# tmathis720/kryst

Hardware: AMD Instinct MI355X
Metric: cg_iterations_per_sec (higher is better)
Workload: dtype f64; 1 GPU; cg_poisson7_512^3; grid=512, rows=134217728, nnz=937951232, partition=1 k-slab(s), rhs=A*1, x0=0, spmv_encoding=csr-p16, launcher=SoloGroup

## Files before the change

### bindings/rust/src/ffi.rs

```rust
#![allow(non_camel_case_types, dead_code)]
use std::os::raw::{c_char, c_void};

pub type Ctx = *mut c_void;
pub type Csr = *mut c_void;
pub type Vecd = *mut c_void;
pub type Pc = *mut c_void;
pub type Session = *mut c_void;
pub type HostFactors = *mut c_void;
pub type HostAmg = *mut c_void;

pub const KRYST_OK: i32 = 0;
pub const KRYST_FACTOR_ERROR: i32 = 1;
pub const KRYST_SOLVE_ERROR: i32 = 2;
pub const KRYST_INDEFINITE_MATRIX: i32 = 3;
pub const KRYST_INDEFINITE_PRECONDITIONER: i32 = 4;
pub const KRYST_ZERO_PIVOT: i32 = 5;
pub const KRYST_UNSUPPORTED: i32 = 6;
pub const KRYST_ERR_HIP: i32 = 100;
pub const KRYST_ERR_RCCL: i32 = 101;
pub const KRYST_ERR_ARG: i32 = 102;
pub const KRYST_ERR_CSR: i32 = 103;
pub const KRYST_ERR_BUSY: i32 = 104;

pub const KRYST_ILU_KRYST_COMPAT: i32 = 0;
// ... 47 lines not shown
    pub fn kryst_ctx_synchronize(ctx: Ctx) -> i32;
    pub fn kryst_ctx_rank(ctx: Ctx, rank: *mut i32, nranks: *mut i32) -> i32;
    pub fn kryst_comm_barrier(ctx: Ctx) -> i32;
    pub fn kryst_comm_all_reduce(ctx: Ctx, x: f64, out: *mut f64) -> i32;
    pub fn kryst_ctx_scalar_reduce(ctx: Ctx, mode: i32, active: *mut i32) -> i32;
    pub fn kryst_csr_halo_mode(a: Csr, mode: i32, active: *mut i32) -> i32;
    pub fn kryst_ctx_trim(ctx: Ctx, bytes_released: *mut i64) -> i32;
    pub fn kryst_phase_timing_begin(ctx: Ctx) -> i32;
    pub fn kryst_phase_timing_end(ctx: Ctx, ms: *mut f64, count: i32) -> i32;
    pub fn kryst_phase_count() -> i32;
    pub fn kryst_phase_name(phase: i32) -> *const c_char;
    pub fn kryst_ctx_timer_start(ctx: Ctx) -> i32;
    pub fn kryst_ctx_timer_stop(ctx: Ctx, ms: *mut f64) -> i32;

    pub fn kryst_vec_create(ctx: Ctx, n: i64, out: *mut Vecd) -> i32;
    pub fn kryst_vec_destroy(v: Vecd) -> i32;
    pub fn kryst_vec_len(v: Vecd, n: *mut i64) -> i32;
    pub fn kryst_vec_upload(v: Vecd, host: *const f64, n: i64) -> i32;
    pub fn kryst_vec_download(v: Vecd, host: *mut f64, n: i64) -> i32;
    pub fn kryst_vec_fill(v: Vecd, value: f64) -> i32;
    pub fn kryst_vec_copy(dst: Vecd, src: Vecd) -> i32;
    pub fn kryst_vec_fill_splitmix(v: Vecd, seed: u64, global_offset: i64) -> i32;

    pub fn kryst_csr_create(ctx: Ctx, nrows: i64, ncols: i64, row_ptr: *const u64, col_idx: *const u64, vals: *const f64, out: *mut Csr) -> i32;
    pub fn kryst_csr_create_i32(ctx: Ctx, nrows: i64, ncols: i64, row_ptr: *const i64, col_idx: *const i32, vals: *const f64, out: *mut Csr) -> i32;
    pub fn kryst_csr_create_dist(ctx: Ctx, n_global: i64, row_offsets: *const i64, row_ptr: *const i64, col_idx_global: *const i64,
                                 vals: *const f64, out: *mut Csr) -> i32;
    pub fn kryst_csr_create_stencil7(ctx: Ctx, n: i32, kind: i32, out: *mut Csr) -> i32;
    pub fn kryst_csr_destroy(a: Csr) -> i32;
    pub fn kryst_csr_shape(a: Csr, nrows_local: *mut i64, ncols_global: *mut i64, nnz_local: *mut i64) -> i32;
    pub fn kryst_csr_encoding(a: Csr, encoding: *mut i32, patterns: *mut i32, table_entries: *mut i32) -> i32;
    pub fn kryst_csr_tile_order(a: Csr, info: *mut i64) -> i32;
    pub fn kryst_csr_pattern_info(a: Csr, info: *mut i64) -> i32;
    pub fn kryst_csr_download(a: Csr, row_ptr: *mut i64, col_idx_local: *mut i32, vals: *mut f64) -> i32;
    pub fn kryst_csr_placement_info(a: Csr, tries: *mut i32, chosen: *mut i32, skeleton_ms8: *mut f64) -> i32;

    pub fn kryst_spmv(a: Csr, x: Vecd, y: Vecd) -> i32;
    pub fn kryst_spmv_transpose(a: Csr, x: Vecd, y: Vecd) -> i32;
    pub fn kryst_spmv_host(a: Csr, x: *const f64, nx: i64, y: *mut f64, ny: i64) -> i32;
    pub fn kryst_bench_spmv(a: Csr, x: Vecd, y: Vecd, fused_dots: i32, reps: i32, avg_ms: *mut f64) -> i32;
    pub fn kryst_bench_streams(ctx: Ctx, n: i64, stride_bytes: i64, kind: i32, reps: i32, avg_ms: *mut f64) -> i32;
    pub fn kryst_bench_csr_skeleton(a: Csr, x: Vecd, y: Vecd, reps: i32, avg_ms: *mut f64) -> i32;
    pub fn kryst_bench_spmv_fused(a: Csr, x: Vecd, y: Vecd, reps: i32, avg_ms: *mut f64) -> i32;
    pub fn kryst_bench_poison_lds(ctx: Ctx) -> i32;
    pub fn kryst_bench_vec_padding(v: Vecd, fill: *const f64, dirty: *mut i64) -> i32;

    pub fn kryst_dot(x: Vecd, y: Vecd, out: *mut f64) -> i32;
    pub fn kryst_norm(x: Vecd, out: *mut f64) -> i32;
    pub fn kryst_axpy(alpha: f64, x: Vecd, y: Vecd) -> i32;
    pub fn kryst_aypx(beta: f64, x: Vecd, y: Vecd) -> i32;
    pub fn kryst_sub(a: Vecd, b: Vecd, out: Vecd) -> i32;

    pub fn kryst_pc_identity(ctx: Ctx, out: *mut Pc) -> i32;
    pub fn kryst_pc_jacobi(a: Csr, out: *mut Pc) -> i32;
    pub fn kryst_pc_ilu0(a: Csr, mode: i32, out: *mut Pc) -> i32;
    pub fn kryst_pc_ilup(a: Csr, fill: i32, out: *mut Pc) -> i32;
    pub fn kryst_pc_ilut(a: Csr, fill: i32, droptol: f64, out: *mut Pc) -> i32;
    pub fn kryst_pc_chebyshev_stub(ctx: Ctx, degree: i32, out: *mut Pc) -> i32;
    pub fn kryst_pc_chebyshev(a: Csr, alpha: f64, beta: f64, degree: i32, out: *mut Pc) -> i32;
    pub fn kryst_pc_approx_inverse(m: Csr, out: *mut Pc) -> i32;
    pub fn kryst_pc_block_jacobi(a: Csr, blk_ptr: *const i64, blk_idx: *const i64, nblocks: i64, out: *mut Pc) -> i32;
    pub fn kryst_pc_block_jacobi_uniform(a: Csr, bsize: i32, out: *mut Pc) -> i32;
    pub fn kryst_pc_block_jacobi_export(pc: Pc, nnz: *mut i64, row_ptr: *mut i64, col: *mut i32, val: *mut f64) -> i32;
    pub fn kryst_pc_asm(a: Csr, sub_ptr: *const i64, sub_idx: *const i64, nsub: i64, overlap: i32, variant: i32, out: *mut Pc) -> i32;
    pub fn kryst_pc_asm_uniform(a: Csr, nparts: i64, overlap: i32, variant: i32, out: *mut Pc) -> i32;
    pub fn kryst_pc_asm_info(pc: Pc, nsub: *mut i64, ext_rows: *mut i64, max_rows: *mut i32) -> i32;
// ... 73 lines not shown
```

### include/kryst_hip.h

```cpp
#ifndef KRYST_HIP_H
#define KRYST_HIP_H
#include <stdint.h>

#ifdef __cplusplus
extern "C" {
#endif

enum {
    KRYST_OK = 0,
    KRYST_FACTOR_ERROR = 1,
    KRYST_SOLVE_ERROR = 2,
    KRYST_INDEFINITE_MATRIX = 3,
    KRYST_INDEFINITE_PRECONDITIONER = 4,
    KRYST_ZERO_PIVOT = 5,
    KRYST_UNSUPPORTED = 6,
    KRYST_ERR_HIP = 100,
    KRYST_ERR_RCCL = 101,
    KRYST_ERR_ARG = 102,
    KRYST_ERR_CSR = 103,
    KRYST_ERR_BUSY = 104
};

typedef struct kryst_ctx_s* kryst_ctx_t;
typedef struct kryst_csr_s* kryst_csr_t;
// ... 17 lines not shown
int32_t kryst_comm_all_reduce(kryst_ctx_t ctx, double x, double* out);
int32_t kryst_ctx_scalar_reduce(kryst_ctx_t ctx, int32_t mode, int32_t* active);
int32_t kryst_csr_halo_mode(kryst_csr_t a, int32_t mode, int32_t* active);
int32_t kryst_ctx_trim(kryst_ctx_t ctx, int64_t* bytes_released);
int32_t kryst_phase_timing_begin(kryst_ctx_t ctx);
int32_t kryst_phase_timing_end(kryst_ctx_t ctx, double* ms, int32_t count);
int32_t kryst_phase_count(void);
const char* kryst_phase_name(int32_t phase);
int32_t kryst_ctx_timer_start(kryst_ctx_t ctx);
int32_t kryst_ctx_timer_stop(kryst_ctx_t ctx, double* ms);

int32_t kryst_vec_create(kryst_ctx_t ctx, int64_t n, kryst_vec_t* out);
int32_t kryst_vec_destroy(kryst_vec_t v);
int32_t kryst_vec_len(kryst_vec_t v, int64_t* n);
int32_t kryst_vec_upload(kryst_vec_t v, const double* host, int64_t n);
int32_t kryst_vec_download(kryst_vec_t v, double* host, int64_t n);
int32_t kryst_vec_fill(kryst_vec_t v, double value);
int32_t kryst_vec_copy(kryst_vec_t dst, kryst_vec_t src);
int32_t kryst_vec_fill_splitmix(kryst_vec_t v, uint64_t seed, int64_t global_offset);

int32_t kryst_csr_create(kryst_ctx_t ctx, int64_t nrows, int64_t ncols, const uint64_t* row_ptr,
                         const uint64_t* col_idx, const double* vals, kryst_csr_t* out);
int32_t kryst_csr_create_i32(kryst_ctx_t ctx, int64_t nrows, int64_t ncols, const int64_t* row_ptr,
                             const int32_t* col_idx, const double* vals, kryst_csr_t* out);
int32_t kryst_csr_create_dist(kryst_ctx_t ctx, int64_t n_global, const int64_t* row_offsets ,
                              const int64_t* row_ptr, const int64_t* col_idx_global, const double* vals,
                              kryst_csr_t* out);
int32_t kryst_csr_create_stencil7(kryst_ctx_t ctx, int32_t N, int32_t kind, kryst_csr_t* out);
int32_t kryst_csr_destroy(kryst_csr_t a);
int32_t kryst_csr_shape(kryst_csr_t a, int64_t* nrows_local, int64_t* ncols_global, int64_t* nnz_local);
int32_t kryst_csr_encoding(kryst_csr_t a, int32_t* encoding, int32_t* patterns, int32_t* table_entries);
int32_t kryst_csr_tile_order(kryst_csr_t a, int64_t* info);
int32_t kryst_csr_pattern_info(kryst_csr_t a, int64_t* info);
int32_t kryst_csr_download(kryst_csr_t a, int64_t* row_ptr, int32_t* col_idx_local, double* vals);
int32_t kryst_csr_placement_info(kryst_csr_t a, int32_t* tries, int32_t* chosen, double* skeleton_ms8);

int32_t kryst_spmv(kryst_csr_t a, kryst_vec_t x, kryst_vec_t y);
int32_t kryst_spmv_transpose(kryst_csr_t a, kryst_vec_t x, kryst_vec_t y);
int32_t kryst_spmv_host(kryst_csr_t a, const double* x, int64_t nx, double* y, int64_t ny);

int32_t kryst_bench_spmv(kryst_csr_t a, kryst_vec_t x, kryst_vec_t y, int32_t fused_dots, int32_t reps, double* avg_ms);
int32_t kryst_bench_streams(kryst_ctx_t ctx, int64_t n, int64_t stride_bytes, int32_t kind, int32_t reps, double* avg_ms);
int32_t kryst_bench_csr_skeleton(kryst_csr_t a, kryst_vec_t x, kryst_vec_t y, int32_t reps, double* avg_ms);
int32_t kryst_bench_spmv_fused(kryst_csr_t a, kryst_vec_t x, kryst_vec_t y, int32_t reps, double* avg_ms);
int32_t kryst_bench_poison_lds(kryst_ctx_t ctx);
int32_t kryst_bench_vec_padding(kryst_vec_t v, const double* fill, int64_t* dirty);

int32_t kryst_dot(kryst_vec_t x, kryst_vec_t y, double* out);
int32_t kryst_norm(kryst_vec_t x, double* out);
int32_t kryst_axpy(double alpha, kryst_vec_t x, kryst_vec_t y);
int32_t kryst_aypx(double beta, kryst_vec_t x, kryst_vec_t y);
int32_t kryst_sub(kryst_vec_t a, kryst_vec_t b, kryst_vec_t out);

enum { KRYST_ILU_KRYST_COMPAT = 0,
       KRYST_ILU_ILUP0 = 1,
       KRYST_ILU_TRUE_ILU0 = 2 };
int32_t kryst_pc_identity(kryst_ctx_t ctx, kryst_pc_t* out);
int32_t kryst_pc_jacobi(kryst_csr_t a, kryst_pc_t* out);
int32_t kryst_pc_ilu0(kryst_csr_t a, int32_t mode, kryst_pc_t* out);
int32_t kryst_pc_ilup(kryst_csr_t a, int32_t fill, kryst_pc_t* out);
int32_t kryst_pc_ilut(kryst_csr_t a, int32_t fill, double droptol, kryst_pc_t* out);
int32_t kryst_pc_chebyshev_stub(kryst_ctx_t ctx, int32_t degree, kryst_pc_t* out);
int32_t kryst_pc_chebyshev(kryst_csr_t a, double alpha, double beta, int32_t degree, kryst_pc_t* out);
int32_t kryst_pc_approx_inverse(kryst_csr_t m, kryst_pc_t* out);
int32_t kryst_pc_block_jacobi(kryst_csr_t a, const int64_t* blk_ptr, const int64_t* blk_idx, int64_t nblocks, kryst_pc_t* out);
int32_t kryst_pc_block_jacobi_uniform(kryst_csr_t a, int32_t bsize, kryst_pc_t* out);
// ... 123 lines not shown
```

### kryst_amd/__init__.py

```python
import ctypes as C
import enum
import numpy as np

from . import _ffi
from ._ffi import KError, lib, check

__all__ = ["Context", "DeviceVec", "CsrMatrix", "dot", "norm", "Jacobi", "Ilu0", "Ilup", "Ilut", "TrueIlu0", "Chebyshev",
           "ChebyshevPc", "IdentityPc", "ApproxInv", "BlockJacobi", "AdditiveSchwarz", "Sor", "MatSorType", "SparsityPattern", "Spai", "Amg", "apply_chebyshev", "Convergence", "SolveStats", "CgNormType",
           "Preconditioning", "CgSolver", "PcgSolver", "GmresSolver", "FgmresSolver", "PcaGmresSolver", "Orthog", "CgsSolver", "TfqmrSolver", "MinresSolver", "QmrSolver", "CgnrSolver", "CgneSolver", "BiCgStabSolver", "BiCgStabRightPcSolver", "Session", "KspContext", "SolverKind", "PC", "KError", "reduce_spec",
           "host_stencil7", "partition_rows", "halo_recv_plan", "read_matrix_market", "read_petsc_binary", "host_ilup", "host_ilut", "host_amg", "host_levels", "color_graph", "build_blocks_from_colors"]


def _dp(a):
    return a.ctypes.data_as(_ffi.c_dp)


def _f64(a):
    return np.ascontiguousarray(a, dtype=np.float64)


def reduce_spec():
    t, v, f = C.c_int32(), C.c_int32(), C.c_int32()
    lib().kryst_reduce_spec(C.byref(t), C.byref(v), C.byref(f))
    return t.value, v.value, f.value
# ... 250 lines not shown

    def spmv_transpose(self, x, y=None):
        if isinstance(x, DeviceVec):
            if y is None:
                y = DeviceVec(self.ctx, self._ncols)
            check(lib().kryst_spmv_transpose(self.h, x.h, y.h))
            return y
        xv = DeviceVec(self.ctx, _f64(x))
        yv = DeviceVec(self.ctx, self._ncols)
        check(lib().kryst_spmv_transpose(self.h, xv.h, yv.h))
        if y is None:
            return yv.to_host()
        if len(y) != self._ncols:
            raise KError(102, "spmv_transpose: y.len() != ncols")
        y[:] = yv.to_host()
        return y

    ENCODINGS = ("csr", "csr-d8", "csr-d16", "csr-p16", "csr-dia")

    def encoding(self):
        e, p, t = C.c_int32(0), C.c_int32(0), C.c_int32(0)
        check(lib().kryst_csr_encoding(self.h, C.byref(e), C.byref(p), C.byref(t)))
        return self.ENCODINGS[e.value], p.value, t.value

    def tile_order(self):
        info = (C.c_int64 * 4)()
        check(lib().kryst_csr_tile_order(self.h, info))
        return {"plane_rows": info[0], "slots": info[1], "slots8": info[2], "in_use": bool(info[3])}

    def pattern_info(self):
        info = (C.c_int64 * 4)()
        check(lib().kryst_csr_pattern_info(self.h, info))
        return {"line": info[0], "uniform_far": bool(info[1]), "interior_first": info[2], "staged": bool(info[3])}

    def placement_info(self):
        t, c = C.c_int32(0), C.c_int32(0)
        ms = (C.c_double * 8)()
        check(lib().kryst_csr_placement_info(self.h, C.byref(t), C.byref(c), ms))
        return {"tries": t.value, "chosen": c.value, "skeleton_ms": [ms[k] for k in range(t.value)]}

    def bench_spmv(self, x, y, fused_dots=1, reps=50):
        ms = C.c_double()
        check(lib().kryst_bench_spmv(self.h, x.h, y.h, fused_dots, reps, C.byref(ms)))
        return ms.value

    def bench_spmv_fused(self, x, y, reps=20):
        ms = C.c_double()
        rc = lib().kryst_bench_spmv_fused(self.h, x.h, y.h, reps, C.byref(ms))
        if rc == 6:
            return None
        check(rc)
        return ms.value

    def halo_mode(self, mode):
        active = C.c_int32(0)
        rc = lib().kryst_csr_halo_mode(self.h, {"rccl": 0, "peer": 1, "query": -1}[mode], C.byref(active))
        if rc not in (0, 6):
            check(rc)
        return "peer" if active.value == 1 else "rccl"

    def bench_csr_skeleton(self, x, y, reps=10):
        ms = C.c_double()
        check(lib().kryst_bench_csr_skeleton(self.h, x.h, y.h, reps, C.byref(ms)))
        return ms.value

    matvec = spmv
# ... 1075 lines not shown
```

### kryst_amd/_ffi.py

```python
import ctypes as C
import os

_HERE = os.path.dirname(os.path.abspath(__file__))
LIB_PATH = os.environ.get("KRYST_HIP_LIB") or os.path.join(_HERE, "lib", "libkryst_hip.so")

OK = 0
ERR_NAMES = {1: "FactorError", 2: "SolveError", 3: "IndefiniteMatrix", 4: "IndefinitePreconditioner",
             5: "ZeroPivot", 6: "Unsupported", 100: "HipError", 101: "RcclError", 102: "ArgumentError",
             103: "CsrError", 104: "ContextBusy"}

c_dp = C.POINTER(C.c_double)
c_i64p = C.POINTER(C.c_int64)
c_u64p = C.POINTER(C.c_uint64)
c_i32p = C.POINTER(C.c_int32)
Handle = C.c_void_p
MONITOR = C.CFUNCTYPE(None, C.c_int64, C.c_double, C.c_void_p)


class Params(C.Structure):
    _fields_ = [("tol", C.c_double), ("max_iters", C.c_int64), ("restart", C.c_int32),
                ("precond_side", C.c_int32), ("norm_type", C.c_int32), ("single_reduction", C.c_int32),
                ("has_radius", C.c_int32), ("radius", C.c_double),
                ("has_obj_target", C.c_int32), ("obj_target", C.c_double), ("check_every", C.c_int32)]

# ... 19 lines not shown
    "kryst_comm_barrier": (C.c_int32, [Handle]),
    "kryst_comm_all_reduce": (C.c_int32, [Handle, C.c_double, c_dp]),
    "kryst_ctx_scalar_reduce": (C.c_int32, [Handle, C.c_int32, c_i32p]),
    "kryst_csr_halo_mode": (C.c_int32, [Handle, C.c_int32, c_i32p]),
    "kryst_ctx_trim": (C.c_int32, [Handle, c_i64p]),
    "kryst_phase_timing_begin": (C.c_int32, [Handle]),
    "kryst_phase_timing_end": (C.c_int32, [Handle, c_dp, C.c_int32]),
    "kryst_phase_count": (C.c_int32, []),
    "kryst_phase_name": (C.c_char_p, [C.c_int32]),
    "kryst_ctx_timer_start": (C.c_int32, [Handle]),
    "kryst_ctx_timer_stop": (C.c_int32, [Handle, c_dp]),
    "kryst_vec_create": (C.c_int32, [Handle, C.c_int64, C.POINTER(Handle)]),
    "kryst_vec_destroy": (C.c_int32, [Handle]),
    "kryst_vec_len": (C.c_int32, [Handle, c_i64p]),
    "kryst_vec_upload": (C.c_int32, [Handle, c_dp, C.c_int64]),
    "kryst_vec_download": (C.c_int32, [Handle, c_dp, C.c_int64]),
    "kryst_vec_fill": (C.c_int32, [Handle, C.c_double]),
    "kryst_vec_copy": (C.c_int32, [Handle, Handle]),
    "kryst_vec_fill_splitmix": (C.c_int32, [Handle, C.c_uint64, C.c_int64]),
    "kryst_csr_create": (C.c_int32, [Handle, C.c_int64, C.c_int64, c_u64p, c_u64p, c_dp, C.POINTER(Handle)]),
    "kryst_csr_create_i32": (C.c_int32, [Handle, C.c_int64, C.c_int64, c_i64p, c_i32p, c_dp, C.POINTER(Handle)]),
    "kryst_csr_create_dist": (C.c_int32, [Handle, C.c_int64, c_i64p, c_i64p, c_i64p, c_dp, C.POINTER(Handle)]),
    "kryst_csr_create_stencil7": (C.c_int32, [Handle, C.c_int32, C.c_int32, C.POINTER(Handle)]),
    "kryst_csr_destroy": (C.c_int32, [Handle]),
    "kryst_csr_shape": (C.c_int32, [Handle, c_i64p, c_i64p, c_i64p]),
    "kryst_csr_download": (C.c_int32, [Handle, c_i64p, c_i32p, c_dp]),
    "kryst_csr_placement_info": (C.c_int32, [Handle, c_i32p, c_i32p, c_dp]),
    "kryst_spmv": (C.c_int32, [Handle, Handle, Handle]),
    "kryst_spmv_host": (C.c_int32, [Handle, c_dp, C.c_int64, c_dp, C.c_int64]),
    "kryst_spmv_transpose": (C.c_int32, [Handle, Handle, Handle]),
    "kryst_csr_encoding": (C.c_int32, [Handle, C.POINTER(C.c_int32), C.POINTER(C.c_int32), C.POINTER(C.c_int32)]),
    "kryst_csr_tile_order": (C.c_int32, [Handle, C.POINTER(C.c_int64)]),
    "kryst_csr_pattern_info": (C.c_int32, [Handle, C.POINTER(C.c_int64)]),
    "kryst_bench_spmv": (C.c_int32, [Handle, Handle, Handle, C.c_int32, C.c_int32, c_dp]),
    "kryst_bench_streams": (C.c_int32, [Handle, C.c_int64, C.c_int64, C.c_int32, C.c_int32, c_dp]),
    "kryst_bench_csr_skeleton": (C.c_int32, [Handle, Handle, Handle, C.c_int32, c_dp]),
    "kryst_bench_spmv_fused": (C.c_int32, [Handle, Handle, Handle, C.c_int32, c_dp]),
    "kryst_bench_poison_lds": (C.c_int32, [Handle]),
    "kryst_bench_vec_padding": (C.c_int32, [Handle, c_dp, c_i64p]),
    "kryst_dot": (C.c_int32, [Handle, Handle, c_dp]),
    "kryst_norm": (C.c_int32, [Handle, c_dp]),
    "kryst_axpy": (C.c_int32, [C.c_double, Handle, Handle]),
    "kryst_aypx": (C.c_int32, [C.c_double, Handle, Handle]),
    "kryst_sub": (C.c_int32, [Handle, Handle, Handle]),
    "kryst_pc_identity": (C.c_int32, [Handle, C.POINTER(Handle)]),
    "kryst_pc_jacobi": (C.c_int32, [Handle, C.POINTER(Handle)]),
    "kryst_pc_ilu0": (C.c_int32, [Handle, C.c_int32, C.POINTER(Handle)]),
    "kryst_pc_ilup": (C.c_int32, [Handle, C.c_int32, C.POINTER(Handle)]),
    "kryst_pc_ilut": (C.c_int32, [Handle, C.c_int32, C.c_double, C.POINTER(Handle)]),
    "kryst_pc_chebyshev_stub": (C.c_int32, [Handle, C.c_int32, C.POINTER(Handle)]),
    "kryst_pc_chebyshev": (C.c_int32, [Handle, C.c_double, C.c_double, C.c_int32, C.POINTER(Handle)]),
    "kryst_pc_approx_inverse": (C.c_int32, [Handle, C.POINTER(Handle)]),
    "kryst_pc_block_jacobi": (C.c_int32, [Handle, c_i64p, c_i64p, C.c_int64, C.POINTER(Handle)]),
    "kryst_pc_block_jacobi_uniform": (C.c_int32, [Handle, C.c_int32, C.POINTER(Handle)]),
    "kryst_pc_block_jacobi_export": (C.c_int32, [Handle, c_i64p, c_i64p, c_i32p, c_dp]),
    "kryst_pc_asm": (C.c_int32, [Handle, c_i64p, c_i64p, C.c_int64, C.c_int32, C.c_int32, C.POINTER(Handle)]),
    "kryst_pc_asm_uniform": (C.c_int32, [Handle, C.c_int64, C.c_int32, C.c_int32, C.POINTER(Handle)]),
    "kryst_pc_asm_info": (C.c_int32, [Handle, c_i64p, c_i64p, c_i32p]),
    "kryst_pc_asm_export": (C.c_int32, [Handle, c_i64p, c_i32p, c_i32p, c_dp]),
    "kryst_pc_sor": (C.c_int32, [Handle, C.c_double, C.c_int64, C.c_int64, C.c_uint32, C.c_double, c_i32p, C.POINTER(Handle)]),
    "kryst_pc_sor_info": (C.c_int32, [Handle, c_i32p, c_i32p, c_i64p, c_i32p, c_i32p]),
    "kryst_pc_spai": (C.c_int32, [Handle, C.c_int32, c_i64p, c_i64p, C.c_int64, C.c_double, C.POINTER(Handle)]),
    "kryst_pc_spai_export": (C.c_int32, [Handle, c_i64p, c_i64p, c_i32p, c_dp]),
    "kryst_pc_amg": (C.c_int32, [Handle, C.c_int32, C.c_double, C.c_int32, C.c_int32, C.c_int32, C.POINTER(Handle)]),
    "kryst_pc_amg_info": (C.c_int32, [Handle, c_i32p, c_i64p, c_i64p, C.c_int32]),
    "kryst_pc_amg_export": (C.c_int32, [Handle, C.c_int32, C.c_int32, c_i64p, c_i64p, c_i64p, c_i64p, c_i32p, c_dp]),
# ... 111 lines not shown
```

### kryst_amd/csrc/spmv.hip

```cpp
#include "csr.h"
#include "ew.h"
#include <algorithm>


namespace kr {

typedef int    v2i __attribute__((ext_vector_type(2)));
typedef double v2d __attribute__((ext_vector_type(2)));

struct SpmvArgs {
    const int32_t* row_ptr; const int32_t* col; const double* val;
    const double* x; const double* halo; int32_t nloc;
    double* y; const int32_t* tiles; int32_t ntiles; int32_t nrows;
    const double* dvec; double* partials; int64_t pstride;
    const int* done; int32_t xcd_chunk; int32_t swizzle; int32_t group;
    const uint8_t* code; const int32_t* dict;
    const uint16_t* code16; const double* vdict;
    const uint16_t* pid; const uint32_t* pmeta; const int32_t* poff; const double* pval; int32_t npat, ntab;
    int32_t pat_red_off;
    int32_t nloc8;
    int32_t tpw;
    int32_t amask;
    const double* dia; int64_t dia_stride; int32_t dia_nd; int32_t dia_min;
    int64_t xsafe; int32_t cmax;
// ... 595 lines not shown
        if constexpr (NQ > 0) {
            double acc[NQ];
            d2 d;
            if constexpr (CENTER) { d.a = B.x; d.b = B.y; } else d = dv[k];
            acc[0] = 0.0;
            if (va) acc[0] = acc[0] + d.a * s0;
            if (vb) acc[0] = acc[0] + d.b * s1;
            if constexpr (NQ > 1) {
                acc[1] = 0.0;
                if (va) acc[1] = acc[1] + s0 * s0;
                if (vb) acc[1] = acc[1] + s1 * s1;
            }
#pragma unroll
            for (int kk = 0; kk < NQ; ++kk) {
                const double wsum = wave_butterfly(acc[kk]);
                if ((t & 63) == 0) red[(k * NQ + kk) * (KR_T / 64) + (t >> 6)] = wsum;
            }
        }
    }
    if constexpr (NQ > 0) {
        __syncthreads();
        if (t < nt * NQ) {
            const int k = t / NQ, kk = t % NQ;
            double sum = red[t * (KR_T / 64)];
#pragma unroll
            for (int w2 = 1; w2 < KR_T / 64; ++w2) sum = sum + red[t * (KR_T / 64) + w2];
            a.partials[kk * a.pstride + q0 + k] = sum;
        }
    }
}

struct FuseArgs { const double* z; const double* p_old; double* p_new; double* xvec; const double* alpha; const double* beta; const long long* xpend; long long it; };
template <int NQ, int T, int NMAX, bool XU>
__global__ __launch_bounds__(KR_T) void spmv_pattern_fuse_kernel(const SpmvArgs a, const FuseArgs f, const int32_t n, const int32_t far_lo, const int32_t far_hi) {
    const bool ended = a.done && *a.done;
    const bool owed = XU && *f.xpend == f.it - 1;
    if (ended && !owed) return;
    extern __shared__ __attribute__((aligned(16))) unsigned char smem[];
    const int XS = T * KR_TILE + 2 * n + 4;
    double* xs = reinterpret_cast<double*>(smem);
    uint2* meta = reinterpret_cast<uint2*>(xs + XS);
    double* pval = reinterpret_cast<double*>(meta + a.npat);
    double* red = reinterpret_cast<double*>(smem + a.pat_red_off);
    const int t = threadIdx.x;
    const int xcd = blockIdx.x & 7, slot = blockIdx.x >> 3;
    const int G = a.group;
    const int qr = (((slot / G) * 8 + xcd) * G + slot % G) * T;
    if (qr >= a.ntiles) return;
    const int nt = min(T, a.ntiles - qr);
    const int q0 = qr;
    const int32_t r0 = q0 * KR_TILE;
    const double al = *f.alpha, be = *f.beta;
    if (ended) {
#pragma unroll
        for (int k = 0; k < T; ++k) {
            if (k >= nt) break;
            const int32_t row = r0 + k * KR_TILE + 2 * t;
            const d2 pp = ld2(f.p_old, row), xx = ld2(f.xvec, row);
            st2(f.xvec, row, xx.a + al * pp.a, xx.b + al * pp.b);
        }
        return;
    }
    unsigned ids[T];
#pragma unroll
    for (int k = 0; k < T; ++k) ids[k] = k < nt ? __builtin_nontemporal_load(reinterpret_cast<const unsigned*>(a.pid + (size_t)(q0 + k) * KR_TILE + 2 * t)) : 0u;
    constexpr int NP = (T * KR_TILE + 2 * NMAX + 4 + 2 * KR_T - 1) / (2 * KR_T);
    const int npairs = XS / 2;
    const int32_t e0 = r0 - n - 2;
    const int32_t xsafe = (int32_t)a.xsafe;
    const bool inside = e0 >= 0 && e0 + XS <= xsafe && (int64_t)r0 + far_lo >= 0 && (int64_t)r0 + T * KR_TILE + far_hi <= (int64_t)xsafe;
    const int own_lo = (n + 2) / 2, own_hi = own_lo + nt * (KR_TILE / 2);
// ... 610 lines not shown
        a->halo_pushed_inline = inl;
        a->halo_started_for = x;
        return KRYST_OK;
    }
    KR_HIP(hipEventRecord(ctx->ev_x_ready, ctx->s_main));
    KR_HIP(hipStreamWaitEvent(ctx->s_comm, ctx->ev_x_ready, 0));
    const void* sendbase = pl.d_sendbuf;
    if (a->send_contiguous) {
        sendbase = x;
    } else if (pl.total_send > 0) {
        hipLaunchKernelGGL(pack_kernel, dim3((unsigned)((pl.total_send + 255) / 256)), dim3(256), 0, ctx->s_comm,
                           x, pl.d_send_idx, pl.d_sendbuf, pl.total_send);
        KR_HIP(hipGetLastError());
    }
    KR_TRY(comm_exchange(ctx, sendbase, pl.send_counts.data(), pl.send_off.data(), pl.d_halo, pl.recv_counts.data(),
                         pl.recv_off.data(), true, ctx->s_comm));
    KR_HIP(hipEventRecord(ctx->ev_halo_done, ctx->s_comm));
    a->halo_started_for = x;
    return KRYST_OK;
}

bool spmv_can_fuse_direction(kryst_csr_t a) {
    return !a->dist && a->d_pid && a->pat_stage_n > 0 && a->pat_far_uniform && a->npat <= 512 && a->ntab <= 512 && a->nrows == a->xlen &&
           takes_pattern_path(a, false) && env_int("KRYST_SPMV_STAGE", 1) != 0 && env_int("KRYST_SPMV_STAGE_UFAR", 1) != 0 &&
           a->xlen + 2 * KR_TILE < (1ll << 31) &&
           env_int("KRYST_CG_FUSE_P", a->nrows * 8 > env_ll("KRYST_CG_FUSE_MIN_BYTES", 768ll << 20) ? 1 : 0) != 0;
}
static int32_t launch_spmv_fused_impl(kryst_csr_t a, const double* z, const double* p_old, double* p_new, double* xvec, double* y, int nq,
                                      const double* alpha, const double* beta, const long long* xpend, long long it, const int* done, bool force);
int32_t launch_spmv_fused(kryst_csr_t a, const double* z, const double* p_old, double* p_new, double* xvec, double* y, int nq,
                          const double* alpha, const double* beta, const long long* xpend, long long it, const int* done) {
    return launch_spmv_fused_impl(a, z, p_old, p_new, xvec, y, nq, alpha, beta, xpend, it, done, false);
}
static int32_t launch_spmv_fused_impl(kryst_csr_t a, const double* z, const double* p_old, double* p_new, double* xvec, double* y, int nq,
                                      const double* alpha, const double* beta, const long long* xpend, long long it, const int* done, bool force) {
    kryst_ctx_t ctx = a->ctx;
    KR_ARG((force || spmv_can_fuse_direction(a)) && nq >= 1 && nq <= 2, "launch_spmv_fused: operator cannot take the fused form");
    KR_TRY(ensure_partials(ctx, a->ntiles));
    SpmvArgs args;
    memset(&args, 0, sizeof args);
    args.x = p_new; args.y = y; args.ntiles = (int32_t)a->ntiles; args.nrows = (int32_t)a->nrows; args.nloc = (int32_t)a->nrows;
    args.dvec = p_new; args.partials = ctx->d_partials; args.pstride = ctx->partials_cap; args.done = done;
    args.pid = a->d_pid; args.pmeta = a->d_pmeta; args.poff = a->d_poff; args.pval = a->d_pval; args.npat = a->npat; args.ntab = a->ntab;
    const int T = env_int("KRYST_SPMV_FUSE_T", 4) <= 2 ? 2 : 4;
    const int32_t n_ = a->pat_stage_n;
    const size_t xs_bytes = sizeof(double) * (size_t)(T * KR_TILE + 2 * n_ + 4);
    const size_t tab = xs_bytes + (size_t)a->npat * 8 + (size_t)a->ntab * 8;
    args.pat_red_off = (int32_t)((tab + 15) & ~(size_t)15);
    size_t lds_s = (size_t)args.pat_red_off + sizeof(double) * (size_t)T * (size_t)nq * (KR_T / 64);
    const int wgcu = env_int("KRYST_SPMV_FUSE_WG_PER_CU", 0);
    if (wgcu > 0) lds_s = std::max(lds_s, std::min<size_t>((size_t)(160 << 10) / (size_t)wgcu - 512, (size_t)64 << 10));
    args.xsafe = (a->xlen + KR_TILE - 1) / KR_TILE * KR_TILE + KR_TILE - 2;
    const int64_t nruns = (a->ntiles + T - 1) / T;
    args.group = std::max(1, env_int("KRYST_SPMV_STAGE_GROUP", stage_group_default(a, nruns, T, true)));
    const int64_t per_xcd = ((nruns + 7) / 8 + args.group - 1) / args.group * args.group;
    const dim3 sgrid((unsigned)(per_xcd * 8)), block(KR_T);
    const FuseArgs f{z, p_old, p_new, xvec, alpha, beta, xpend, it};
#ifdef KR_TUNING
    args.abl = env_int("KRYST_FUSE_ABL", 0);
#endif
    if (lds_s > ((size_t)48 << 10)) {
        static bool raised = false;
        if (!raised) {
#define KR_FUSE_FNS(NQ_, T_, X_) (const void*)spmv_pattern_fuse_kernel<NQ_, T_, 512, X_>, (const void*)spmv_pattern_fuse_kernel<NQ_, T_, 1024, X_>
            for (const void* fn : {KR_FUSE_FNS(1, 2, true), KR_FUSE_FNS(1, 4, true), KR_FUSE_FNS(2, 2, true), KR_FUSE_FNS(2, 4, true),
                                   KR_FUSE_FNS(1, 2, false), KR_FUSE_FNS(1, 4, false), KR_FUSE_FNS(2, 2, false), KR_FUSE_FNS(2, 4, false)})
                (void)hipFuncSetAttribute(fn, hipFuncAttributeMaxDynamicSharedMemorySize, 64 << 10);
#undef KR_FUSE_FNS
            raised = true;
        }
    }
#define KR_FUSE_N(NQ_, T_, X_) do { if (n_ <= 512) hipLaunchKernelGGL((spmv_pattern_fuse_kernel<NQ_, T_, 512, X_>), sgrid, block, lds_s, ctx->s_main, args, f, n_, a->pat_far_lo, a->pat_far_hi); \
                                    else hipLaunchKernelGGL((spmv_pattern_fuse_kernel<NQ_, T_, 1024, X_>), sgrid, block, lds_s, ctx->s_main, args, f, n_, a->pat_far_lo, a->pat_far_hi); } while (0)
#define KR_FUSE(NQ_) do { if (xvec) { if (T == 2) KR_FUSE_N(NQ_, 2, true); else KR_FUSE_N(NQ_, 4, true); } \
                          else { if (T == 2) KR_FUSE_N(NQ_, 2, false); else KR_FUSE_N(NQ_, 4, false); } } while (0)
    if (nq == 1) KR_FUSE(1); else KR_FUSE(2);
#undef KR_FUSE
#undef KR_FUSE_N
    KR_HIP(hipGetLastError());
    phase_mark(ctx, KR_PH_SPMV);
    return KRYST_OK;
}

static int32_t halo_finish(kryst_csr_t a, int budget) {
    kryst_ctx_t ctx = a->ctx;
    if (a->plan.peer.on) {
        HaloPeer& hp = a->plan.peer;
        if (!a->halo_pushed_inline) KR_HIP(hipStreamWaitEvent(ctx->s_main, ctx->ev_halo_done, 0));
        if (hp.npull > 0) {
            static const int dflt = [] { const char* e = getenv("KRYST_IPC_POLL_BUDGET"); return e ? std::max(1, atoi(e)) : (1 << 26); }();
            const unsigned gx = (unsigned)std::min<int64_t>(std::max<int64_t>(1, (hp.pull_max + 1023) / 1024), 256);
            hipLaunchKernelGGL(halo_pull_kernel, dim3(gx, (unsigned)hp.npull), dim3(256), 0, ctx->s_main, hp.landing + (size_t)(hp.epoch & 1ull) * hp.stride,
                               a->plan.d_halo, hp.d_pull, hp.epoch, budget > 0 ? std::min(budget, dflt) : dflt, fold_err(ctx) + 1);
// ... 62 lines not shown
}

int32_t kryst_spmv(kryst_csr_t a, kryst_vec_t x, kryst_vec_t y) {
    KR_ARG(a && x && y, "spmv");
    KR_ARG(x->ctx == a->ctx && y->ctx == a->ctx, "spmv: context mismatch");
    KR_ARG(x->n == a->xlen, "spmv: x.len() != ncols");
    KR_ARG(y->n == a->nrows, "spmv: y.len() != nrows");
    KR_ARG(x->d != y->d, "spmv: x and y alias");
    KR_HIP(hipSetDevice(a->ctx->device));
    KR_TRY(launch_spmv(a, x->d, y->d, 0, nullptr, nullptr));
    if (a->dist && a->plan.peer.on && use_collectives(a->ctx) && fold_gave_up(a->ctx)) return KRYST_ERR_RCCL;
    return KRYST_OK;
}

int32_t kryst_csr_encoding(kryst_csr_t a, int32_t* encoding, int32_t* patterns, int32_t* table_entries) {
    KR_ARG(a && encoding, "csr_encoding");
    const int lvl = env_int("KRYST_SPMV_COMPRESS", 3);
    int e = 0;
    const bool p16_fits = a->xlen + a->plan.total_recv < (1ll << 28) && a->nrows < (1ll << 28);
    if (a->d_pid && lvl >= 3 && p16_fits) e = 3;
    else if (a->d_code16 && lvl >= 2) e = 2;
    else if (a->d_dia && lvl >= 1 && env_int("KRYST_SPMV_DIA", 1) != 0) e = 4;
    else if (a->d_code && lvl >= 1) e = 1;
    *encoding = e;
    if (patterns) *patterns = e == 4 ? a->dia_nd : (a->d_pid ? a->npat : 0);
    if (table_entries) *table_entries = a->d_pid ? a->ntab : 0;
    return KRYST_OK;
}

int32_t kryst_csr_tile_order(kryst_csr_t a, int64_t* info) {
    KR_ARG(a && info, "csr_tile_order");
    info[0] = a->d_tile_order ? a->order_plane : 0; info[1] = a->order_slots1; info[2] = a->order_slots8;
    info[3] = uses_tile_order(a) ? 1 : 0;
    return KRYST_OK;
}

int32_t kryst_csr_pattern_info(kryst_csr_t a, int64_t* info) {
    KR_ARG(a && info, "csr_pattern_info");
    info[0] = a->d_pid ? a->pat_stage_n : 0; info[1] = a->pat_far_uniform ? 1 : 0; info[2] = a->interior_first;
    info[3] = (a->d_pid && a->pat_stage_n > 0 && takes_pattern_path(a, false) && a->npat <= 512 && a->ntab <= 512 && env_int("KRYST_SPMV_STAGE", 1) != 0 &&
               a->xlen + 2 * KR_TILE < (1ll << 31) && (!a->dist || !use_collectives(a->ctx) || a->interior_first >= 0)) ? 1 : 0;
    return KRYST_OK;
}

int32_t kryst_bench_spmv(kryst_csr_t a, kryst_vec_t x, kryst_vec_t y, int32_t fused_dots, int32_t reps, double* avg_ms) {
    KR_ARG(a && x && y && avg_ms && reps >= 1 && fused_dots >= 0 && fused_dots <= 2, "bench_spmv");
    KR_ARG(x->n == a->xlen && y->n == a->nrows, "bench_spmv: size mismatch");
    KR_ARG(fused_dots == 0 || a->nrows == a->xlen, "bench_spmv: fused dots need a square operator");
    kryst_ctx_t ctx = a->ctx;
    KR_HIP(hipSetDevice(ctx->device));
    const size_t bytes = sizeof(double) * (size_t)((x->n + KR_TILE - 1) / KR_TILE * KR_TILE + KR_TILE);
    double* xs[3] = {x->d, nullptr, nullptr};
    for (int k = 1; k < 3; ++k) {
        if (hipMalloc(&xs[k], bytes) != hipSuccess) { (void)hipGetLastError(); xs[k] = x->d; continue; }
        KR_HIP(hipMemcpyAsync(xs[k], x->d, bytes, hipMemcpyDeviceToDevice, ctx->s_main));
    }
    int32_t rc = launch_spmv(a, xs[0], y->d, fused_dots, xs[0], nullptr);
    (void)hipEventRecord(ctx->tm0, ctx->s_main);
    for (int r = 0; r < reps && rc == KRYST_OK; ++r) rc = launch_spmv(a, xs[(r + 1) % 3], y->d, fused_dots, xs[(r + 1) % 3], nullptr);
    (void)hipEventRecord(ctx->tm1, ctx->s_main);
    (void)hipEventSynchronize(ctx->tm1);
    float ms = 0.f;
    (void)hipEventElapsedTime(&ms, ctx->tm0, ctx->tm1);
    *avg_ms = (double)ms / reps;
    (void)hipStreamSynchronize(ctx->s_main);
    if (use_collectives(ctx)) (void)hipStreamSynchronize(ctx->s_comm);
// ... 53 lines not shown
```

Before: 609.5 iterations/s.

## Add plane-marching fused SpMV kernel reusing z-plane windows in LDS

Adds a marching variant of the fused CG SpMV kernel. Each workgroup owns a strip of a k-plane and walks S consecutive planes, keeping a double-buffered LDS window of the recomputed p vector. The k-1 and k+1 neighbours come from registers and the next plane's window, so the p/z halo for the z-direction is not reloaded. It is enabled by default for large uniform-stencil operators, at the cost of more LDS, fewer workgroups and an extra barrier per plane.

```diff
diff --git a/bindings/rust/src/ffi.rs b/bindings/rust/src/ffi.rs
--- a/bindings/rust/src/ffi.rs
+++ b/bindings/rust/src/ffi.rs
@@ -103,6 +103,7 @@
     pub fn kryst_csr_encoding(a: Csr, encoding: *mut i32, patterns: *mut i32, table_entries: *mut i32) -> i32;
     pub fn kryst_csr_tile_order(a: Csr, info: *mut i64) -> i32;
     pub fn kryst_csr_pattern_info(a: Csr, info: *mut i64) -> i32;
+    pub fn kryst_csr_fuse_march_info(a: Csr, info: *mut i64) -> i32;
     pub fn kryst_csr_download(a: Csr, row_ptr: *mut i64, col_idx_local: *mut i32, vals: *mut f64) -> i32;
     pub fn kryst_csr_placement_info(a: Csr, tries: *mut i32, chosen: *mut i32, skeleton_ms8: *mut f64) -> i32;
 
diff --git a/include/kryst_hip.h b/include/kryst_hip.h
--- a/include/kryst_hip.h
+++ b/include/kryst_hip.h
@@ -73,6 +73,7 @@
 int32_t kryst_csr_encoding(kryst_csr_t a, int32_t* encoding, int32_t* patterns, int32_t* table_entries);
 int32_t kryst_csr_tile_order(kryst_csr_t a, int64_t* info);
 int32_t kryst_csr_pattern_info(kryst_csr_t a, int64_t* info);
+int32_t kryst_csr_fuse_march_info(kryst_csr_t a, int64_t* info);
 int32_t kryst_csr_download(kryst_csr_t a, int64_t* row_ptr, int32_t* col_idx_local, double* vals);
 int32_t kryst_csr_placement_info(kryst_csr_t a, int32_t* tries, int32_t* chosen, double* skeleton_ms8);
 
diff --git a/kryst_amd/__init__.py b/kryst_amd/__init__.py
--- a/kryst_amd/__init__.py
+++ b/kryst_amd/__init__.py
@@ -306,6 +306,11 @@
         info = (C.c_int64 * 4)()
         check(lib().kryst_csr_pattern_info(self.h, info))
         return {"line": info[0], "uniform_far": bool(info[1]), "interior_first": info[2], "staged": bool(info[3])}
+
+    def fuse_march_info(self):
+        info = (C.c_int64 * 6)()
+        check(lib().kryst_csr_fuse_march_info(self.h, info))
+        return {"eligible": bool(info[0]), "on": bool(info[1]), "T": info[2], "strips": info[3], "S": info[4], "segments": info[5]}
 
     def placement_info(self):
         t, c = C.c_int32(0), C.c_int32(0)
diff --git a/kryst_amd/_ffi.py b/kryst_amd/_ffi.py
--- a/kryst_amd/_ffi.py
+++ b/kryst_amd/_ffi.py
@@ -75,6 +75,7 @@
     "kryst_csr_encoding": (C.c_int32, [Handle, C.POINTER(C.c_int32), C.POINTER(C.c_int32), C.POINTER(C.c_int32)]),
     "kryst_csr_tile_order": (C.c_int32, [Handle, C.POINTER(C.c_int64)]),
     "kryst_csr_pattern_info": (C.c_int32, [Handle, C.POINTER(C.c_int64)]),
+    "kryst_csr_fuse_march_info": (C.c_int32, [Handle, C.POINTER(C.c_int64)]),
     "kryst_bench_spmv": (C.c_int32, [Handle, Handle, Handle, C.c_int32, C.c_int32, c_dp]),
     "kryst_bench_streams": (C.c_int32, [Handle, C.c_int64, C.c_int64, C.c_int32, C.c_int32, c_dp]),
     "kryst_bench_csr_skeleton": (C.c_int32, [Handle, Handle, Handle, C.c_int32, c_dp]),
diff --git a/kryst_amd/csrc/spmv.hip b/kryst_amd/csrc/spmv.hip
--- a/kryst_amd/csrc/spmv.hip
+++ b/kryst_amd/csrc/spmv.hip
@@ -651,11 +651,158 @@
 
 struct FuseArgs { const double* z; const double* p_old; double* p_new; double* xvec; const double* alpha; const double* beta; const long long* xpend; long long it; };
 template <int NQ, int T, int NMAX, bool XU>
+__device__ __forceinline__ void fuse_march(const SpmvArgs& a, const FuseArgs& f, const int32_t n, const int32_t plane, unsigned char* smem, const bool ended, const bool owed) {
+    const int XS = T * KR_TILE + 2 * n + 4;
+    double* win = reinterpret_cast<double*>(smem);
+    uint2* meta = reinterpret_cast<uint2*>(win + 2 * XS);
+    double* pval = reinterpret_cast<double*>(meta + a.npat);
+    double* red = reinterpret_cast<double*>(smem + a.pat_red_off);
+    const int t = threadIdx.x;
+    const int xcd = blockIdx.x & 7, slot = blockIdx.x >> 3;
+    const int spx = a.group, S = a.xcd_chunk;
+    const int strip = xcd * spx + slot % spx, k0 = (slot / spx) * S;
+    const int nplanes = a.nrows / plane;
+    if (strip >= a.tpw || k0 >= nplanes) return;
+    const int ns = min(S, nplanes - k0);
+    const int32_t rbeg = k0 * plane + strip * (T * KR_TILE);
+    const double al = *f.alpha, be = *f.beta;
+    if (ended) {
+        for (int s = 0; s < ns; ++s) {
+#pragma unroll
+            for (int k = 0; k < T; ++k) {
+                const int32_t row = rbeg + s * plane + k * KR_TILE + 2 * t;
+                const d2 pp = ld2(f.p_old, row), xx = ld2(f.xvec, row);
+                st2(f.xvec, row, xx.a + al * pp.a, xx.b + al * pp.b);
+            }
+        }
+        return;
+    }
+    constexpr int NP = (T * KR_TILE + 2 * NMAX + 4 + 2 * KR_T - 1) / (2 * KR_T);
+    const int npairs = XS / 2;
+    const int32_t xsafe = (int32_t)a.xsafe;
+    const int own_lo = (n + 2) / 2, own_hi = own_lo + T * (KR_TILE / 2);
+    v2d zz[NP], po[NP], xo[XU ? NP : 1];
+    auto request = [&](const int32_t r0) {
+        const int32_t e0 = r0 - n - 2;
+        const bool inside = e0 >= 0 && e0 + XS <= xsafe;
+#pragma unroll
+        for (int i = 0; i < NP; ++i) {
+            const int pi = min(t + i * KR_T, npairs - 1);
+            const int32_t e = inside ? e0 + 2 * pi : min(max(e0 + 2 * pi, 0), xsafe);
+            po[i] = *reinterpret_cast<const v2d*>(f.p_old + e);
+            zz[i] = *reinterpret_cast<const v2d*>(f.z + e);
+            if constexpr (XU) { xo[i].x = 0.0; xo[i].y = 0.0; if (owed && pi >= own_lo && pi < own_hi) xo[i] = __builtin_nontemporal_load(reinterpret_cast<const v2d*>(f.xvec + e)); }
+        }
+    };
+    auto write_window = [&](const int32_t r0, double* xs) {
+        const int32_t e0 = r0 - n - 2;
+#pragma unroll
+        for (int i = 0; i < NP; ++i) {
+            const int pi = t + i * KR_T;
+            if (pi < npairs) {
+                v2d pn; pn.x = zz[i].x + be * po[i].x; pn.y = zz[i].y + be * po[i].y;
+                *reinterpret_cast<v2d*>(xs + 2 * pi) = pn;
+                if (pi >= own_lo && pi < own_hi) {
+                    const int32_t row = e0 + 2 * pi;
+                    st2(f.p_new, row, pn.x, pn.y);
+                    if constexpr (XU) { if (owed) st2(f.xvec, row, xo[i].x + al * po[i].x, xo[i].y + al * po[i].y); }
+                }
+            }
+        }
+    };
+    auto far_pair = [&](const int64_t row) {
+        const int64_t c = min(max(row, (int64_t)0), (int64_t)xsafe);
+        const v2d zf = *reinterpret_cast<const v2d*>(f.z + c), pf = *reinterpret_cast<const v2d*>(f.p_old + c);
+        v2d r; r.x = zf.x + be * pf.x; r.y = zf.y + be * pf.y;
+        return r;
+    };
+    unsigned ids[T], idn[T];
+    v2d prev[T], hi[T];
+#pragma unroll
+    for (int k = 0; k < T; ++k) { ids[k] = __builtin_nontemporal_load(reinterpret_cast<const unsigned*>(a.pid + (size_t)rbeg + k * KR_TILE + 2 * t)); idn[k] = 0u; }
+    double* w0 = win; double* w1 = win + XS;
+    request(rbeg);
+#pragma unroll
+    for (int k = 0; k < T; ++k) { prev[k] = far_pair((int64_t)rbeg + k * KR_TILE + 2 * t - plane); hi[k].x = 0.0; hi[k].y = 0.0; }
+    for (int i = t; i < a.npat; i += KR_T) meta[i] = reinterpret_cast<const uint2*>(a.pmeta)[i];
+    for (int i = t; i < a.ntab; i += KR_T) pval[i] = a.pval[i];
+    write_window(rbeg, w0);
+    if (ns > 1) {
+        request(rbeg + plane);
+        write_window(rbeg + plane, w1);
+    }
+    __syncthreads();
+    for (int s = 0; s < ns; ++s) {
+        const int32_t r0 = rbeg + s * plane;
+        const bool last = s + 1 == ns, fill = s + 2 < ns;
+        if (fill) request(r0 + 2 * plane);
+        if (!last) {
+#pragma unroll
+            for (int k = 0; k < T; ++k) idn[k] = __builtin_nontemporal_load(reinterpret_cast<const unsigned*>(a.pid + (size_t)(r0 + plane) + k * KR_TILE + 2 * t));
+        } else {
+#pragma unroll
+            for (int k = 0; k < T; ++k) hi[k] = far_pair((int64_t)r0 + k * KR_TILE + 2 * t + plane);
+        }
+#pragma unroll
+        for (int k = 0; k < T; ++k) {
+            const int32_t row = r0 + k * KR_TILE + 2 * t;
+            const uint2 ma = meta[ids[k] & 0xffffu], mb = meta[ids[k] >> 16];
+            const int j = k * KR_TILE + 2 * t + n + 2;
+            const v2d A = *reinterpret_cast<const v2d*>(w0 + j - 2), B = *reinterpret_cast<const v2d*>(w0 + j), C = *reinterpret_cast<const v2d*>(w0 + j + 2);
+            const v2d M = *reinterpret_cast<const v2d*>(w0 + j - n), P = *reinterpret_cast<const v2d*>(w0 + j + n);
+            const v2d U = *reinterpret_cast<const v2d*>(w1 + j);
+            v2d e[7];
+            e[0] = prev[k]; e[1] = M; e[2].x = A.y; e[2].y = B.x; e[3] = B; e[4].x = B.y; e[4].y = C.x; e[5] = P;
+            e[6].x = last ? hi[k].x : U.x; e[6].y = last ? hi[k].y : U.y;
+            prev[k] = B;
+            const double* tva = pval + (ma.x & 0xffffu); const double* tvb = pval + (mb.x & 0xffffu);
+            const unsigned ka = ma.y, kb = mb.y;
+            double s0 = 0.0, s1 = 0.0;
+#pragma unroll
+            for (int u = 0; u < 7; ++u) {
+                const double ta = s0 + tva[u] * e[u].x, tb = s1 + tvb[u] * e[u].y;
+                s0 = ((ka >> u) & 1u) ? ta : s0;
+                s1 = ((kb >> u) & 1u) ? tb : s1;
+            }
+            st2(a.y, row, s0, s1);
+            double acc[NQ];
+            acc[0] = 0.0;
+            acc[0] = acc[0] + B.x * s0;
+            acc[0] = acc[0] + B.y * s1;
+            if constexpr (NQ > 1) {
+                acc[1] = 0.0;
+                acc[1] = acc[1] + s0 * s0;
+                acc[1] = acc[1] + s1 * s1;
+            }
+#pragma unroll
+            for (int kk = 0; kk < NQ; ++kk) {
+                const double wsum = wave_butterfly(acc[kk]);
+                if ((t & 63) == 0) red[(k * NQ + kk) * (KR_T / 64) + (t >> 6)] = wsum;
+            }
+        }
+        __syncthreads();
+        if (t < T * NQ) {
+            const int k = t / NQ, kk = t % NQ;
+            double sum = red[t * (KR_T / 64)];
+#pragma unroll
+            for (int w = 1; w < KR_T / 64; ++w) sum = sum + red[t * (KR_T / 64) + w];
+            a.partials[kk * a.pstride + r0 / KR_TILE + k] = sum;
+        }
+        if (fill) write_window(r0 + 2 * plane, w0);
+        __syncthreads();
+#pragma unroll
+        for (int k = 0; k < T; ++k) ids[k] = idn[k];
+        double* w = w0; w0 = w1; w1 = w;
+    }
+}
+
+template <int NQ, int T, int NMAX, bool XU, bool MARCH = false>
 __global__ __launch_bounds__(KR_T) void spmv_pattern_fuse_kernel(const SpmvArgs a, const FuseArgs f, const int32_t n, const int32_t far_lo, const int32_t far_hi) {
     const bool ended = a.done && *a.done;
     const bool owed = XU && *f.xpend == f.it - 1;
     if (ended && !owed) return;
     extern __shared__ __attribute__((aligned(16))) unsigned char smem[];
+    if constexpr (MARCH) { fuse_march<NQ, T, NMAX, XU>(a, f, n, far_hi, smem, ended, owed); return; }
     const int XS = T * KR_TILE + 2 * n + 4;
     double* xs = reinterpret_cast<double*>(smem);
     uint2* meta = reinterpret_cast<uint2*>(xs + XS);
@@ -1332,6 +1479,32 @@
                           const double* alpha, const double* beta, const long long* xpend, long long it, const int* done) {
     return launch_spmv_fused_impl(a, z, p_old, p_new, xvec, y, nq, alpha, beta, xpend, it, done, false);
 }
+struct FuseMarchPlan { bool eligible, on; int T, strips, S, segs; size_t red_off, lds; };
+static FuseMarchPlan fuse_march_plan(kryst_csr_t a, int nq) {
+    FuseMarchPlan m;
+    memset(&m, 0, sizeof m);
+    m.T = env_int("KRYST_SPMV_FUSE_T", 4) <= 2 ? 2 : 4;
+    const int64_t plane = a->pat_far_uniform ? (int64_t)a->pat_far_hi : 0, R = (int64_t)m.T * KR_TILE;
+    const int32_t n_ = a->pat_stage_n;
+    if (!(a->d_pid && n_ > 0 && n_ <= 512 && plane > 0 && (int64_t)a->pat_far_lo == -plane && plane % R == 0 && a->nrows % plane == 0 && a->nrows == a->xlen)) return m;
+    const size_t tab = 2 * sizeof(double) * (size_t)(R + 2 * n_ + 4) + (size_t)a->npat * 8 + (size_t)a->ntab * 8;
+    m.red_off = (tab + 15) & ~(size_t)15;
+    m.lds = m.red_off + sizeof(double) * (size_t)m.T * (size_t)nq * (KR_T / 64);
+    if (m.lds > ((size_t)80 << 10)) return m;
+    const int64_t nplanes = a->nrows / plane;
+    m.eligible = true;
+    m.strips = (int)(plane / R);
+    int S = env_int("KRYST_SPMV_FUSE_SEG", 0);
+    if (S <= 0) {
+        const int64_t want = std::max<int64_t>(1, (int64_t)a->ctx->num_cu * 4 / m.strips);
+        S = (int)std::max<int64_t>((nplanes + want - 1) / want, std::min<int64_t>(4, nplanes));
+    }
+    m.S = (int)std::min<int64_t>(S, nplanes);
+    m.segs = (int)((nplanes + m.S - 1) / m.S);
+    m.on = env_int("KRYST_SPMV_FUSE_MARCH", a->nrows * 8 > env_ll("KRYST_CG_FUSE_MIN_BYTES", 768ll << 20) ? 1 : 0) != 0;
+    return m;
+}
+
 static int32_t launch_spmv_fused_impl(kryst_csr_t a, const double* z, const double* p_old, double* p_new, double* xvec, double* y, int nq,
                                       const double* alpha, const double* beta, const long long* xpend, long long it, const int* done, bool force) {
     kryst_ctx_t ctx = a->ctx;
@@ -1359,6 +1532,35 @@
 #ifdef KR_TUNING
     args.abl = env_int("KRYST_FUSE_ABL", 0);
 #endif
+    const FuseMarchPlan m = fuse_march_plan(a, 2);
+#ifdef KR_TUNING
+    if (m.eligible && m.on && !args.abl) {
+#else
+    if (m.eligible && m.on) {
+#endif
+        const int spx = (m.strips + 7) / 8;
+        args.group = spx; args.xcd_chunk = m.S; args.tpw = m.strips; args.pat_red_off = (int32_t)m.red_off;
+        size_t lds_m = m.lds;
+        const int wgm = wgcu > 0 ? wgcu : 2;
+        lds_m = std::max(lds_m, std::min<size_t>((size_t)(160 << 10) / (size_t)wgm - 512, (size_t)80 << 10));
+        static bool raised_m = false;
+        if (!raised_m) {
+#define KR_MARCH_FNS(NQ_, T_) (const void*)spmv_pattern_fuse_kernel<NQ_, T_, 512, true, true>, (const void*)spmv_pattern_fuse_kernel<NQ_, T_, 512, false, true>
+            for (const void* fn : {KR_MARCH_FNS(1, 2), KR_MARCH_FNS(1, 4), KR_MARCH_FNS(2, 2), KR_MARCH_FNS(2, 4)})
+                (void)hipFuncSetAttribute(fn, hipFuncAttributeMaxDynamicSharedMemorySize, 80 << 10);
+#undef KR_MARCH_FNS
+            raised_m = true;
+        }
+        const dim3 mgrid((unsigned)(8 * spx * m.segs));
+#define KR_MARCH_X(NQ_, T_) do { if (xvec) hipLaunchKernelGGL((spmv_pattern_fuse_kernel<NQ_, T_, 512, true, true>), mgrid, block, lds_m, ctx->s_main, args, f, n_, a->pat_far_lo, a->pat_far_hi); \
+                                 else hipLaunchKernelGGL((spmv_pattern_fuse_kernel<NQ_, T_, 512, false, true>), mgrid, block, lds_m, ctx->s_main, args, f, n_, a->pat_far_lo, a->pat_far_hi); } while (0)
+        if (nq == 1) { if (T == 2) KR_MARCH_X(1, 2); else KR_MARCH_X(1, 4); }
+        else { if (T == 2) KR_MARCH_X(2, 2); else KR_MARCH_X(2, 4); }
+#undef KR_MARCH_X
+        KR_HIP(hipGetLastError());
+        phase_mark(ctx, KR_PH_SPMV);
+        return KRYST_OK;
+    }
     if (lds_s > ((size_t)48 << 10)) {
         static bool raised = false;
         if (!raised) {
@@ -1487,6 +1689,16 @@
     KR_ARG(a && info, "csr_tile_order");
     info[0] = a->d_tile_order ? a->order_plane : 0; info[1] = a->order_slots1; info[2] = a->order_slots8;
     info[3] = uses_tile_order(a) ? 1 : 0;
+    return KRYST_OK;
+}
+
+int32_t kryst_csr_fuse_march_info(kryst_csr_t a, int64_t* info) {
+    KR_ARG(a && info, "csr_fuse_march_info");
+    const bool form = !a->dist && a->d_pid && a->pat_stage_n > 0 && a->pat_far_uniform && a->npat <= 512 && a->ntab <= 512 && a->nrows == a->xlen && takes_pattern_path(a, false);
+    FuseMarchPlan m;
+    memset(&m, 0, sizeof m);
+    if (form) m = fuse_march_plan(a, 2);
+    info[0] = m.eligible ? 1 : 0; info[1] = m.eligible && m.on ? 1 : 0; info[2] = m.T; info[3] = m.strips; info[4] = m.S; info[5] = m.segs;
     return KRYST_OK;
 }
 
```

Result: faster. 638.7 iterations/s, median of 6 (+4.8%).
